# medivhna/TF_Face_Toolbox

Hardware: NVIDIA B200
Metric: A-softmax head fwd+bwd samples/sec at C=85,742 D=512, 1/2/4/8 B200 (higher is better)
Workload: dtype bf16

## Files before the change

tf_face_toolbox_b200/csrc/asm_api.cu:

```cuda
#include <math.h>
#include <stdio.h>
#include <stdlib.h>
#include <string.h>

#include <new>
#include <vector>

#include "../../include/asoftmax_b200.h"
#include "asm_kernels.cuh"

using namespace asmh;

struct asm_head {
  asm_config cfg;
  int device = 0;
  int num_sms = 148;
  int Cp = 0;
  int NT = 0;
  char* ws = nullptr;
  size_t ws_bytes = 0;
  Step st{};
  size_t dx_part_capacity = 0;
  UmmaMaps maps{};
  int maps_B = -1;
// ... 2 lines not shown
  float* dw_scratch = nullptr;
  bool defer_loss = true;
  bool tc = false;
  UmmaTuning tune{8192, 1024, 2048, 15, 0, 0, 1, 1, 0, 3};
  bool fwd_valid = false;
  cudaStream_t side = nullptr;
  cudaEvent_t ev_fork = nullptr, ev_join = nullptr;
  bool overlap = true;
  int dw_pairs = 0;
  bool pdl = true;
  P2P p2p{};
  bool p2p_ready = false;
  float* Xg = nullptr;
  size_t l2_persist_bytes = 0;
  cudaStream_t l2_stream = nullptr;
  bool l2_set = false;
  int launches = 0;
  bool profiling = false;
  bool phase_profiling = false;
  static constexpr int kMaxMarks = 16;
  cudaEvent_t ev[kMaxMarks + 1] = {};
  const char* mark_name[kMaxMarks] = {};
  int n_marks = 0;
  char err[512];
};

namespace {
thread_local char g_create_err[512] = "";

size_t align_up(size_t v, size_t a) { return (v + a - 1) / a * a; }

struct Layout {
  size_t ylocal, flags, n, inv_n, inv_c, margin, tgt_s, tgt_f, part, stats_local, lse, negoff, gtarget, rcoef, rowloss, counter,
      q_part, G, dx_part, Xb, Wb, Xs, Xg, step_dev, wsq_part, wsq_ticket, total;
  int Cp, NT, MT;
  size_t dx_capacity;
};

bool valid_cfg(const asm_config* c) {
  if (!c) return false;
  if (c->D <= 0 || c->D % 16 != 0) return false;
  if (c->C_total <= 0 || c->C_local <= 0 || c->class_offset < 0) return false;
  if ((long long)c->class_offset + c->C_local > c->C_total) return false;
  if (c->B_max <= 0 || c->m < 1 || c->m > 4) return false;
  if (c->mode != ASM_MODE_FP32 && c->mode != ASM_MODE_BF16) return false;
  if (c->mode == ASM_MODE_BF16 && c->D % 64 != 0) return false;
  if (c->world < 1 || c->rank < 0 || c->rank >= c->world) return false;
  if (c->nccl_comm != nullptr) return false;
  return true;
}

bool use_x3(const asm_config& c) {
  if (c.mode != ASM_MODE_FP32 || c.D % 64 != 0) return false;
  const char* e = getenv("ASM_FP32_SIMT");
  return !(e && atoi(e) != 0);
}
bool use_tc(const asm_config& c) { return c.mode == ASM_MODE_BF16 || use_x3(c); }

Layout make_layout(const asm_config& c, int num_sms) {
  Layout L{};
  const bool tc = use_tc(c);
  const size_t planes = use_x3(c) ? 3 : 1;
  const size_t B = c.B_max, D = c.D;
  L.Cp = (int)align_up(c.C_local, 256);
  L.NT = (L.Cp + 127) / 128;
  if (L.NT < 2 * num_sms) L.NT = 2 * num_sms;
  L.MT = 2 * (int)((B + 127) / 128);
  if (L.MT < 4 * (int)((B + 255) / 256)) L.MT = 4 * (int)((B + 255) / 256);
  const int ks_simt = simt_dx_splits(c.B_max, c.D, L.Cp);
  const int ks_umma = umma_dx_splits(c.B_max, c.D, L.Cp, num_sms, 1);
  const int ks_one = tc ? umma_dx_splits(128, c.D, L.Cp, num_sms, 1)
                        : simt_dx_splits(128, c.D, L.Cp);
  const size_t cap_full = (size_t)(tc ? ks_umma : ks_simt) * B * D;
  const size_t cap_one = (size_t)ks_one * (B < 128 ? B : 128) * D;
  L.dx_capacity = cap_full > cap_one ? cap_full : cap_one;
  size_t off = 0;
  auto take = [&](size_t bytes) { size_t o = off; off = align_up(off + bytes, 256); return o; };
  L.ylocal = take(B * 4);
  L.flags = take(256);
  L.n = take(B * 4);
  L.inv_n = take(B * 4);
  L.inv_c = take((size_t)L.Cp * 4);
  L.margin = take(kMarginRecordFloats * 4);
  L.tgt_s = take(B * 4);
  L.tgt_f = take(B * 4);
  L.part = take(B * (size_t)L.NT * 8);
  L.stats_local = take(3 * B * 4);
  L.lse = take(B * 4);
  L.negoff = take(B * 4);
  L.gtarget = take(B * 4);
  L.rcoef = take(B * 4);
  L.rowloss = take(B * 4);
  L.counter = take(256);
  L.wsq_part = take(((size_t)L.Cp / 32 + 16) * 4);
  L.wsq_ticket = take(256);
  L.q_part = take((size_t)L.MT * L.Cp * 4);
  L.G = take(align_up(B, 64) * (size_t)L.Cp * (c.mode == ASM_MODE_BF16 ? 2 : 4));
  L.dx_part = take(L.dx_capacity * 4);
  if (tc) {
    L.Xb = take(planes * B * D * 2);
    L.Wb = take(planes * D * (size_t)L.Cp * 2);
  } else {
    L.Xs = take(B * D * 4);
  }
  if (c.world > 1) {
    L.Xg = take(B * D * 4);
    L.step_dev = take(256);
  }
  L.total = off;
  return L;
}

int fail(asm_head* h, int code, const char* fmt, const char* detail) {
  char* dst = h ? h->err : g_create_err;
  snprintf(dst, 512, fmt, detail ? detail : "");
  return code;
}

#define CU_TRY(h, expr)                                                         \
  do {                                                                          \
    cudaError_t e__ = (expr);                                                   \
    if (e__ != cudaSuccess) return fail(h, ASM_ERR_CUDA, #expr ": %s", cudaGetErrorString(e__)); \
  } while (0)

void mark(asm_head* h, const char* name, cudaStream_t stream, bool phase_start = true) {
  h->launches += 1;
  if (h->phase_profiling && !phase_start) return;
  if (h->profiling && h->n_marks < asm_head::kMaxMarks) {
    cudaEventRecord(h->ev[h->n_marks], stream);
    h->mark_name[h->n_marks] = name;
    h->n_marks += 1;
  }
}
void mark_end(asm_head* h, cudaStream_t stream) {
  if (h->profiling) cudaEventRecord(h->ev[h->n_marks], stream);
}

int check_launch(asm_head* h, const char* what) {
  cudaError_t e = cudaGetLastError();
  if (e != cudaSuccess) {
    snprintf(h->err, 512, "%s: %s", what, cudaGetErrorString(e));
    return ASM_ERR_CUDA;
  }
  return ASM_OK;
}

bool split_active(const asm_head* h) {
  return h->dw_pairs > 0 && h->overlap && (!h->profiling || h->phase_profiling) && h->side != nullptr && h->tc &&
         (h->tune.cg_mask & 12) == 12;
}
int dw_sms(const asm_head* h) { return split_active(h) ? 2 * h->dw_pairs : h->num_sms; }
int dx_sms(const asm_head* h) { return split_active(h) ? h->num_sms - 2 * h->dw_pairs : h->num_sms; }

Step simt_step(const Step& s) {
  Step t = s;
  if (s.mg.kind != 0) t.X = s.Xs;
  return t;
}

int run_forward(asm_head* h, const float* X, int B, const void* labels, int label_bytes,
                const float* W, float lambda, float* logits, bool want_local_stats,
                cudaStream_t stream, const P2P* tp = nullptr) {
  if (!h) return ASM_ERR_INVALID_ARG;
  if (!X || !labels || !W) return fail(h, ASM_ERR_INVALID_ARG, "null input pointer%s", "");
  if (B <= 0 || B > h->cfg.B_max) return fail(h, ASM_ERR_INVALID_ARG, "B out of range%s", "");
  if (label_bytes != 4 && label_bytes != 8)
    return fail(h, ASM_ERR_INVALID_ARG, "label_bytes must be 4 or 8%s", "");
  if (!(lambda >= 0.f)) return fail(h, ASM_ERR_INVALID_ARG, "lambda must be >= 0%s", "");
  Step& s = h->st;
  s.B = B;
  s.lambda = lambda;
  s.invB = 1.0f / (float)B;
  s.Bp = (int)align_up((size_t)B, 64);
  s.X = X;
  s.W = W;
  s.logits = logits;
  s.l2_hints = (h->tune.l2_hints & 1) ? 1 : 0;
  {
    const int bcg = (h->tune.cg_mask & 2) ? 2 : 1;
    const long long bunits = (long long)(s.Cp / (128 * bcg)) * ((B + 255) / 256);
    s.MT = h->tc ? umma_q_parts(B, umma_tile_width(h->tune, bcg, bunits, h->num_sms), bcg)
                 : (B + kRowTileHost - 1) / kRowTileHost;
  }
  h->launches = 0;
  h->n_marks = 0;
  {
    cudaStreamCaptureStatus cs = cudaStreamCaptureStatusNone;
    cudaStreamIsCapturing(stream, &cs);
    s.pdl = (h->pdl && !h->profiling && cs == cudaStreamCaptureStatusNone) ? 1 : 0;
  }
  h->fwd_valid = false;
  if (h->l2_persist_bytes && h->cfg.mode == ASM_MODE_BF16 && (!h->l2_set || h->l2_stream != stream)) {
    cudaDeviceSetLimit(cudaLimitPersistingL2CacheSize, h->l2_persist_bytes);
    cudaStreamAttrValue av{};
    const size_t wb_bytes = (size_t)s.D * s.Cp * 2;
    av.accessPolicyWindow.base_ptr = (void*)s.Wb;
    av.accessPolicyWindow.num_bytes = wb_bytes;
    av.accessPolicyWindow.hitRatio =
        wb_bytes <= h->l2_persist_bytes ? 1.0f : (float)h->l2_persist_bytes / (float)wb_bytes;
    av.accessPolicyWindow.hitProp = cudaAccessPropertyPersisting;
    av.accessPolicyWindow.missProp = cudaAccessPropertyStreaming;
    if (cudaStreamSetAttribute(stream, cudaStreamAttributeAccessPolicyWindow, &av) != cudaSuccess)
      cudaGetLastError();
    h->l2_set = true;
    h->l2_stream = stream;
  }
  if (h->tc) {
    if ((B + 127) / 128 > h->num_sms)
      return fail(h, ASM_ERR_INVALID_ARG, "batch too large for the tcgen05 forward grid%s", "");
    {
      const int fcg = (h->tune.cg_mask & 1) ? 2 : 1;
      const int ecg = (fcg == 2 && B > 128) ? 2 : 1;
      const long long funits = (long long)(((B + 127) / 128 + ecg - 1) / ecg) * (s.Cp / 256);
      s.NT = umma_forward_tiles(B, s.Cp, h->num_sms, fcg, umma_tile_width(h->tune, ecg, funits, h->num_sms));
    }
    s.KS = umma_dx_splits(B, s.D, s.Cp, dx_sms(h), (h->tune.cg_mask & 8) ? 2 : 1);
    while (s.KS > 1 && (size_t)s.KS * B * s.D > h->dx_part_capacity) --s.KS;
    if (h->maps_B != B || h->maps_KS != s.KS) {
      if (!umma_build_maps(&h->maps, s))
        return fail(h, ASM_ERR_CUDA, "cuTensorMapEncodeTiled failed%s", "");
      h->maps_B = B;
      h->maps_KS = s.KS;
    }
  } else {
    s.NT = simt_forward_tiles(s.C);
    s.KS = simt_dx_splits(B, s.D, s.Cp);
  }
  while (s.KS > 1 && (size_t)s.KS * B * s.D > h->dx_part_capacity) --s.KS;
  mark(h, "prep_norms", stream);
  launch_prep(s, labels, label_bytes, stream, tp);
  mark(h, "fwd_logits_stats", stream);
  if (h->tc) launch_umma_forward(s, h->maps, h->tune, h->num_sms, stream);
  else launch_simt_forward(simt_step(s), stream);
  if (want_local_stats) {
    mark(h, "combine_local", stream);
    launch_combine_local(s, stream);
  }
  mark_end(h, stream);
  int rc = check_launch(h, "forward launch");
  if (rc == ASM_OK) h->fwd_valid = true;
  return rc;
}

int run_backward(asm_head* h, const float* stats_all, int n_shards, float* loss_out,
                 float* dX, float* dW, bool grads, cudaStream_t stream, const P2P* tp = nullptr) {
  Step& s = h->st;
  s.loss = loss_out;
  s.dX = dX;
  s.dW = dW;
  s.Wmut = const_cast<float*>(s.W);
  const bool tc = h->tc;
  s.defer_loss = (grads && tc && h->defer_loss) ? 1 : 0;
  if (tp) {
    mark(h, "combine_exchange", stream);
    launch_combine_p2p(s, *tp, stream);
  } else if (stats_all) {
    if (h->profiling && h->n_marks > 0 && h->n_marks < asm_head::kMaxMarks)
      h->mark_name[h->n_marks++] = "stats_exchange_host";
    mark(h, "combine_global", stream);
    launch_combine_global(s, stats_all, n_shards, stream);
  } else {
    mark(h, "combine_stats", stream);
    launch_combine_fused(s, stream);
  }
  if (grads) {
    h->tune.side_by_side = split_active(h) ? 1 : 0;
    mark(h, "bwd_recompute_g", stream);
    if (tc) launch_umma_bwdg(s, h->maps, h->tune, h->num_sms, stream);
    else launch_simt_bwdg(simt_step(s), stream);
    const bool dx_first = !tc && s.opt.kind != 0;
    const bool fork = h->overlap && (!h->profiling || h->phase_profiling) && h->side != nullptr && !dx_first;
    cudaStream_t sx = stream;
    if (fork) {
      cudaEventRecord(h->ev_fork, stream);
      cudaStreamWaitEvent(h->side, h->ev_fork, 0);
      sx = h->side;
    }
    auto run_dx = [&]() {
      mark(h, "dx_gemm", sx, !h->phase_profiling);
      if (tc) launch_umma_dx(s, h->maps, h->tune, dx_sms(h), sx);
      else launch_simt_dx(simt_step(s), sx);
      const bool add = s.mg.kind != 0;
      mark(h, tp ? (add ? "dx_finish_margin_exchange" : "dx_finish_exchange") : (add ? "dx_finish_margin" : "dx_finish"), sx,
           !h->phase_profiling);
      if (tp) launch_dx_finish_p2p(s, *tp, sx);
      else launch_dx_finish(s, sx);
    };
    if (dx_first) run_dx();
    mark(h, h->phase_profiling ? "dw+dx+dx_finish (side by side)" : "dw_gemm", stream);
    if (tc && s.opt.kind != 0 && h->opt_stream) {
      if (!h->dw_scratch &&
          cudaMalloc(&h->dw_scratch, (size_t)s.D * h->cfg.C_local * sizeof(float)) != cudaSuccess) {
        cudaGetLastError();
        h->dw_scratch = nullptr;
// ... 102 lines not shown
    ce = umma_configure();
    if (ce != cudaSuccess) {
      fail(nullptr, ASM_ERR_CUDA, "cudaFuncSetAttribute(smem): %s", cudaGetErrorString(ce));
      cudaFree(h->ws);
      delete h;
      return ASM_ERR_CUDA;
    }
  }
  Step& s = h->st;
  s.D = cfg->D;
  s.C = cfg->C_local;
  s.Cp = L.Cp;
  s.C_total = cfg->C_total;
  s.class_offset = cfg->class_offset;
  s.m = cfg->m;
  s.mode = cfg->mode;
  s.x3 = use_x3(*cfg) ? 1 : 0;
  char* w = h->ws;
  s.ylocal = (int*)(w + L.ylocal);
  s.flags = (int*)(w + L.flags);
  s.n = (float*)(w + L.n);
  s.inv_n = (float*)(w + L.inv_n);
  s.inv_c = (float*)(w + L.inv_c);
  s.tgt_s = (float*)(w + L.tgt_s);
  s.tgt_f = (float*)(w + L.tgt_f);
  s.part = (float2*)(w + L.part);
  s.stats_local = (float*)(w + L.stats_local);
  s.lse = (float*)(w + L.lse);
  s.negoff = (float*)(w + L.negoff);
  s.gtarget = (float*)(w + L.gtarget);
  s.rcoef = (float*)(w + L.rcoef);
  s.rowloss = (float*)(w + L.rowloss);
  s.counter = (unsigned int*)(w + L.counter);
  s.q_part = (float*)(w + L.q_part);
  s.wsq_part = (float*)(w + L.wsq_part);
  s.wsq_ticket = (unsigned int*)(w + L.wsq_ticket);
  s.gscale = 1.0f;
  s.wd_g = 0.0f;
  s.reg_scale = 0.0f;
  s.reg_out = nullptr;
  s.G = (void*)(w + L.G);
  s.dx_part = (float*)(w + L.dx_part);
  h->dx_part_capacity = L.dx_capacity;
  if (h->tc) {
    s.Xb = (__nv_bfloat16*)(w + L.Xb);
    s.Wb = (__nv_bfloat16*)(w + L.Wb);
  } else {
    s.Xs = (float*)(w + L.Xs);
  }
  s.mg.kind = 0;
  if (cfg->world > 1) {
    h->Xg = (float*)(w + L.Xg);
    h->p2p.step_dev = (unsigned*)(w + L.step_dev);
    h->p2p.err_dev = h->p2p.step_dev + 1;
    h->p2p.tickets = h->p2p.step_dev + 2;
  }
  h->Cp = L.Cp;
  *out = h;
  return ASM_OK;
}

int asm_destroy(asm_head* h) {
  if (!h) return ASM_ERR_INVALID_ARG;
  if (h->ws) cudaFree(h->ws);
  if (h->dw_scratch) cudaFree(h->dw_scratch);
  if (h->side) cudaStreamDestroy(h->side);
  if (h->ev_fork) cudaEventDestroy(h->ev_fork);
  if (h->ev_join) cudaEventDestroy(h->ev_join);
  if (h->ev[0])
    for (int i = 0; i <= asm_head::kMaxMarks; ++i) cudaEventDestroy(h->ev[i]);
  delete h;
  return ASM_OK;
}

const char* asm_last_error(const asm_head* h) { return h ? h->err : g_create_err; }

int asm_last_launch_count(const asm_head* h) { return h ? h->launches : 0; }

int asm_forward_partial(asm_head* h, const float* X, int32_t B, const void* labels,
                        int32_t label_bytes, const float* W, float lambda, float* stats_out,
                        float* logits_out_or_null, void* cuda_stream) {
  cudaStream_t stream = (cudaStream_t)cuda_stream;
  int rc = run_forward(h, X, B, labels, label_bytes, W, lambda, logits_out_or_null, true, stream);
  if (rc != ASM_OK) return rc;
  if (!stats_out) return fail(h, ASM_ERR_INVALID_ARG, "stats_out is NULL%s", "");
  CU_TRY(h, cudaMemcpyAsync(stats_out, h->st.stats_local, (size_t)3 * B * sizeof(float),
                            cudaMemcpyDeviceToDevice, stream));
  return ASM_OK;
}

int asm_backward_partial(asm_head* h, const float* stats_all, int32_t n_shards, float* loss_out,
                         float* dX_partial, float* dW, void* cuda_stream) {
  if (!h) return ASM_ERR_INVALID_ARG;
  if (!h->fwd_valid)
    return fail(h, ASM_ERR_INVALID_ARG, "asm_backward_partial without asm_forward_partial%s", "");
  if (!stats_all || n_shards < 1 || !dX_partial || (!dW && h->st.opt.kind == 0))
    return fail(h, ASM_ERR_INVALID_ARG, "null pointer / bad n_shards%s", "");
  return run_backward(h, stats_all, n_shards, loss_out, dX_partial, dW, true,
                      (cudaStream_t)cuda_stream);
}

int asm_forward_backward(asm_head* h, const float* X, int32_t B, const void* labels,
                         int32_t label_bytes, const float* W, float lambda, float* loss_out,
                         float* logits_out_or_null, float* dX, float* dW, void* cuda_stream) {
  cudaStream_t stream = (cudaStream_t)cuda_stream;
  if (h && h->cfg.C_local != h->cfg.C_total)
    return fail(h, ASM_ERR_INVALID_ARG,
                "asm_forward_backward needs a shard that owns every class; use the partial calls%s", "");
  int rc = run_forward(h, X, B, labels, label_bytes, W, lambda, logits_out_or_null, false, stream);
  if (rc != ASM_OK) return rc;
  if (!loss_out || !dX || (!dW && h->st.opt.kind == 0))
    return fail(h, ASM_ERR_INVALID_ARG, "null output pointer%s", "");
  return run_backward(h, nullptr, 1, loss_out, dX, dW, true, stream);
}

int asm_forward(asm_head* h, const float* X, int32_t B, const void* labels, int32_t label_bytes,
                const float* W, float lambda, float* loss_out, float* logits_out_or_null,
                void* cuda_stream) {
  cudaStream_t stream = (cudaStream_t)cuda_stream;
  if (h && h->cfg.C_local != h->cfg.C_total)
    return fail(h, ASM_ERR_INVALID_ARG, "asm_forward needs a shard that owns every class%s", "");
  int rc = run_forward(h, X, B, labels, label_bytes, W, lambda, logits_out_or_null, false, stream);
  if (rc != ASM_OK) return rc;
  if (!loss_out) return fail(h, ASM_ERR_INVALID_ARG, "loss_out is NULL%s", "");
  return run_backward(h, nullptr, 1, loss_out, nullptr, nullptr, false, stream);
}

namespace {
struct P2PLayout { size_t off_x, off_y, off_st, off_dx, off_fl, total; int b_max; };
P2PLayout p2p_layout(const asm_config& c) {
  P2PLayout L{};
  const size_t B = c.B_max, D = c.D;
  L.b_max = (int)((B + c.world - 1) / c.world);
  size_t off = 0;
  auto take = [&](size_t bytes) { size_t o = off; off = align_up(off + bytes, 256); return o; };
  L.off_x = take(2 * (size_t)L.b_max * D * 4);
  L.off_y = take(2 * (size_t)L.b_max * 4);
  L.off_st = take(2 * 3 * B * 4);
  L.off_dx = take(2 * B * D * 4);
  L.off_fl = take(3 * kFlagStride * 4);
  L.total = off;
  return L;
}
}

size_t asm_p2p_bytes(const asm_config* cfg) {
  if (!valid_cfg(cfg) || cfg->world < 2 || cfg->world > kMaxPeers) return 0;
  return p2p_layout(*cfg).total;
}

int asm_p2p_attach(asm_head* h, void* const* peer_bases) {
  if (!h || !peer_bases) return ASM_ERR_INVALID_ARG;
  if (h->cfg.world < 2 || h->cfg.world > kMaxPeers)
    return fail(h, ASM_ERR_INVALID_ARG, "asm_p2p_attach needs 2..8 ranks%s", "");
  const P2PLayout L = p2p_layout(h->cfg);
// ... 8 lines not shown
    if (!peer_bases[r]) return fail(h, ASM_ERR_INVALID_ARG, "peer base is NULL%s", "");
    p.base[r] = (char*)peer_bases[r];
  }
  const char* e = getenv("ASM_P2P_TIMEOUT_MS");
  p.timeout_ns = (unsigned long long)(e ? atoll(e) : 60000ll) * 1000000ull;
  e = getenv("ASM_P2P_WAITERS");
  p.waiters = e ? atoi(e) : 1 << 20;
  if (p.waiters < 1) p.waiters = 1;
  p2p_preload_kernels();
  h->p2p_ready = true;
  return ASM_OK;
}

int asm_step_p2p(asm_head* h, const float* X_local, int32_t b_local, const void* labels_local,
                 int32_t label_bytes, const float* W, float lambda, float* loss_out,
                 float* dX_local, float* dW, void* cuda_stream) {
  if (!h) return ASM_ERR_INVALID_ARG;
  if (!h->p2p_ready) return fail(h, ASM_ERR_INVALID_ARG, "asm_step_p2p before asm_p2p_attach%s", "");
  if (!X_local || !labels_local || !W || !loss_out || !dX_local || (!dW && h->st.opt.kind == 0))
    return fail(h, ASM_ERR_INVALID_ARG, "null pointer%s", "");
  if (label_bytes != 4 && label_bytes != 8)
    return fail(h, ASM_ERR_INVALID_ARG, "label_bytes must be 4 or 8%s", "");
  P2P& p = h->p2p;
  if (b_local <= 0 || b_local > p.b_max || (long long)b_local * p.world > h->cfg.B_max)
    return fail(h, ASM_ERR_INVALID_ARG, "b_local out of range%s", "");
  cudaStream_t stream = (cudaStream_t)cuda_stream;
  p.b_local = b_local;
  p.x_local = X_local;
  p.y_local = labels_local;
  p.y_bytes = label_bytes;
  p.dx_local = dX_local;
  p.Xg = h->Xg;
  const int B = b_local * p.world;
  int rc = run_forward(h, h->Xg, B, labels_local, label_bytes, W, lambda, nullptr, false, stream, &p);
  if (rc == ASM_OK) rc = run_backward(h, nullptr, p.world, loss_out, nullptr, dW, true, stream, &p);
  return rc;
}

int asm_p2p_set_timeout(asm_head* h, int32_t milliseconds) {
  if (!h || milliseconds < 0) return ASM_ERR_INVALID_ARG;
  h->p2p.timeout_ns = (unsigned long long)milliseconds * 1000000ull;
  return ASM_OK;
}

int asm_p2p_status(asm_head* h, void* cuda_stream) {
  if (!h) return ASM_ERR_INVALID_ARG;
  if (!h->p2p_ready) return ASM_OK;
  unsigned code = 0;
  CU_TRY(h, cudaMemcpyAsync(&code, h->p2p.err_dev, sizeof(code), cudaMemcpyDeviceToHost,
                            (cudaStream_t)cuda_stream));
  CU_TRY(h, cudaStreamSynchronize((cudaStream_t)cuda_stream));
  if (code == 0) return ASM_OK;
  snprintf(h->err, sizeof(h->err), "peer %u did not publish phase %u in time (ranks must stay in lock-step)",
           code & 0xffu, (code >> 8) & 0xffu);
  return ASM_ERR_PEER_TIMEOUT;
}

int asm_set_optimizer(asm_head* h, const asm_optimizer* opt, float* state0, float* state1) {
  if (!h) return ASM_ERR_INVALID_ARG;
  Step& s = h->st;
  if (!opt || opt->kind == ASM_OPT_NONE) {
    s.opt.kind = 0;
    s.opt_s0 = s.opt_s1 = nullptr;
    return ASM_OK;
  }
  if (opt->kind != ASM_OPT_MOMENTUM && opt->kind != ASM_OPT_ADAM)
    return fail(h, ASM_ERR_INVALID_ARG, "unknown optimizer kind%s", "");
// ... 112 lines not shown
```

tf_face_toolbox_b200/csrc/asm_kernels.cuh:

```cuda
#pragma once
#include <cuda.h>
#include <cuda_bf16.h>
#include <cuda_runtime.h>
#include <stdint.h>

#include "asm_common.cuh"

namespace asmh {

struct OptParams {
  int kind;
  float lr;
  float mu, b1, b2, eps, wd;
};
__host__ __device__ inline void opt_apply(const OptParams& o, float grad, float& w, float& s0,
                                          float& s1) {
  const float g = grad + o.wd * w;
  if (o.kind == 1) {
    s0 = o.mu * s0 + g;
    w -= o.lr * s0;
  } else {
    s0 = o.b1 * s0 + (1.0f - o.b1) * g;
    s1 = o.b2 * s1 + (1.0f - o.b2) * g * g;
#ifdef __CUDA_ARCH__
// ... 70 lines not shown
struct Step {
  int B, D, C, Cp, C_total, class_offset, m, mode;
  float lambda, invB;
  const float* lambda_dev;
  float gscale;
  float wd_g;
  float reg_scale;
  float* reg_out;
  float* wsq_part;
  unsigned int* wsq_ticket;
  const float* X;
  int x_bf16;
  const float* W;
  float* logits;
  float* dX;
  float* dW;
  float* loss;
  int* ylocal;
  int* flags;
  float* n;
  float* inv_n;
  float* inv_c;
  float* tgt_s;
  float* tgt_f;
  float2* part;
  int NT;
  float* stats_local;
  float* lse;
  float* negoff;
  float* gtarget;
  float* rcoef;
  float* rowloss;
  unsigned int* counter;
  float* q_part;
  int MT;
  void* G;
  int Bp;
  float* dx_part;
  int KS;
  __nv_bfloat16* Xb;
  __nv_bfloat16* Wb;
  int x3;
  OptParams opt;
  float* Wmut;
  float* opt_s0;
  float* opt_s1;
  int l2_hints;
  int pdl;
  int defer_loss;
  Margin mg;
  float* Xs;
};

void launch_prep(const Step& s, const void* labels, int label_bytes, cudaStream_t st, const P2P* p = nullptr);
void launch_combine_p2p(const Step& s, const P2P& p, cudaStream_t st);
void launch_dx_finish_p2p(const Step& s, const P2P& p, cudaStream_t st);
void launch_combine_local(const Step& s, cudaStream_t st);
void launch_combine_global(const Step& s, const float* stats_all, int n_shards, cudaStream_t st);
void launch_combine_fused(const Step& s, cudaStream_t st);
void launch_dx_finish(const Step& s, cudaStream_t st);
void launch_opt_stream(const Step& s, const float* dW, cudaStream_t st);

void p2p_preload_kernels();
void prep_preload_kernels();
void simt_preload_kernels();

// ... 58 lines not shown
```

tf_face_toolbox_b200/csrc/asm_prep.cu:

```cuda
#include <stdlib.h>

#include "asm_common.cuh"
#include "asm_kernels.cuh"
#include "asm_p2p.cuh"
#include "asm_rows.cuh"

namespace asmh {

__device__ __forceinline__ void prep_row_tail(const Step& s, int row, float acc, long long y) {
  const float nn = sqrtf(acc);
  s.n[row] = nn;
  s.inv_n[row] = nn > 0.f ? 1.0f / nn : 0.f;
  const long long yl = y - s.class_offset;
  s.ylocal[row] = (y < 0 || y >= s.C_total) ? -2 : ((yl >= 0 && yl < s.C) ? (int)yl : -1);
  s.tgt_s[row] = 0.f;
  s.tgt_f[row] = 0.f;
}

template <int PL>
__device__ __forceinline__ void prep_row_scaled(const Step& s, const char* x, char* xg, int esz, bool gather,
                                                int row, long long y) {
  const int tx = threadIdx.x & 31;
  const float4* x4 = reinterpret_cast<const float4*>(x);
  const int n16 = s.D * esz / 16;
// ... 281 lines not shown
    if (vec2) prep_kernel<true, 0, TX, TY, U, ADD><<<grd, 256, 0, st>>>(s, labels, label_bytes, nwb, npub, pp);
    else prep_kernel<false, 0, TX, TY, U, ADD><<<grd, 256, 0, st>>>(s, labels, label_bytes, nwb, npub, pp);
  }
}

template <int TX, int TY, int U>
static void launch_prep_t(const Step& s, const void* labels, int label_bytes, cudaStream_t st, const P2P* p) {
  if (s.mg.kind != 0) launch_prep_t<TX, TY, U, true>(s, labels, label_bytes, st, p);
  else launch_prep_t<TX, TY, U, false>(s, labels, label_bytes, st, p);
}

void launch_prep(const Step& s, const void* labels, int label_bytes, cudaStream_t st, const P2P* p) {
  static int shape = -1, small_auto = -1;
  if (shape < 0) {
    const char* e = getenv("ASM_PREP_SHAPE");
    shape = e ? atoi(e) : 0;
    e = getenv("ASM_PREP_AUTO");
    small_auto = (e && atoi(e) != 0) ? 1 : 0;
  }
  if (shape == 0 && small_auto && s.Cp <= 32768) {
    launch_prep_t<16, 16, 8>(s, labels, label_bytes, st, p);
    return;
  }
  if (shape == 1) launch_prep_t<32, 8, 16>(s, labels, label_bytes, st, p);
  else if (shape == 2) launch_prep_t<16, 16, 8>(s, labels, label_bytes, st, p);
  else if (shape == 3) launch_prep_t<128, 2, 16>(s, labels, label_bytes, st, p);
  else launch_prep_t<32, 8, 4>(s, labels, label_bytes, st, p);
}

__global__ void __launch_bounds__(256) combine_local_kernel(Step s) {
  pdl_trigger();
  pdl_wait();
  const int row = blockIdx.x * 8 + (threadIdx.x >> 5);
  const int lane = threadIdx.x & 31;
  if (row >= s.B) return;
  float m = -INFINITY, z = 0.f;
  const float2* p = s.part + (size_t)row * s.NT;
  for (int t = lane; t < s.NT; t += 32) {
    const float2 v = p[t];
    ms_combine(m, z, v.x, v.y);
  }
#pragma unroll
  for (int o = 16; o > 0; o >>= 1) {
    const float m2 = __shfl_xor_sync(0xffffffffu, m, o);
    const float z2 = __shfl_xor_sync(0xffffffffu, z, o);
    ms_combine(m, z, m2, z2);
  }
  if (lane == 0) {
    float* st = s.stats_local;
    st[row] = m;
    st[s.B + row] = z;
    st[2 * s.B + row] = s.ylocal[row] >= 0 ? s.tgt_f[row] : 0.f;
  }
}

void launch_combine_local(const Step& s, cudaStream_t st) {
  launch_pdl(combine_local_kernel, dim3((s.B + 7) / 8), dim3(256), 0, st, s.pdl != 0, 1, s);
}

template <bool FUSED>
__global__ void __launch_bounds__(256) combine_kernel(Step s, const float* stats_all, int n_shards) {
  __shared__ float red[256];
  __shared__ bool is_last;
  pdl_trigger();
  pdl_wait();
  const int row = blockIdx.x * 8 + (threadIdx.x >> 5);
  const int lane = threadIdx.x & 31;
  if (row < s.B) {
    float m = -INFINITY, z = 0.f, fy = 0.f;
    const int yl_row = s.ylocal[row];
    const float tgt_f_row = s.tgt_f[row], tgt_s_row = s.tgt_s[row], inv_n_row = s.inv_n[row];
    if (FUSED) {
      const float2* p = s.part + (size_t)row * s.NT;
      for (int t = lane; t < s.NT; t += 32) {
        const float2 v = p[t];
        ms_combine(m, z, v.x, v.y);
      }
    } else {
      for (int g = lane; g < n_shards; g += 32) {
        const float* sg = stats_all + (size_t)g * 3 * s.B;
        ms_combine(m, z, sg[row], sg[s.B + row]);
        fy += sg[2 * s.B + row];
      }
    }
#pragma unroll
    for (int o = 16; o > 0; o >>= 1) {
      const float m2 = __shfl_xor_sync(0xffffffffu, m, o);
      const float z2 = __shfl_xor_sync(0xffffffffu, z, o);
      ms_combine(m, z, m2, z2);
      fy += __shfl_xor_sync(0xffffffffu, fy, o);
    }
    if (lane == 0) {
      if (FUSED) {
        fy = yl_row >= 0 ? tgt_f_row : 0.f;
        s.stats_local[row] = m;
        s.stats_local[s.B + row] = z;
        s.stats_local[2 * s.B + row] = fy;
      }
      row_epilogue(s, row, m, z, fy, yl_row, tgt_f_row, tgt_s_row, inv_n_row);
    }
  }
  if (s.defer_loss) return;
  last_block_loss(s, red, &is_last);
}

void launch_combine_global(const Step& s, const float* stats_all, int n_shards, cudaStream_t st) {
  launch_pdl(combine_kernel<false>, dim3((s.B + 7) / 8), dim3(256), 0, st, false, 1, s, stats_all, n_shards);
}

void launch_combine_fused(const Step& s, cudaStream_t st) {
  launch_pdl(combine_kernel<true>, dim3((s.B + 7) / 8), dim3(256), 0, st, s.pdl != 0, 1, s,
             static_cast<const float*>(nullptr), 1);
}

template <int KS_T>
__global__ void __launch_bounds__(256) dx_finish_kernel(Step s) {
  pdl_trigger();
  pdl_wait();
  dx_finish_rows<KS_T>(s, s.dX, blockIdx.x, gridDim.x);
}

__global__ void __launch_bounds__(256) dx_finish_margin_kernel(Step s) {
  __shared__ float red[8];
  pdl_trigger();
  pdl_wait();
  dx_finish_rows_margin(s, s.dX, blockIdx.x, gridDim.x, red);
}

void launch_dx_finish(const Step& s, cudaStream_t st) {
  if (s.mg.kind != 0) {
    int blocks = (s.B + 1) / 2;
    if (blocks > 148 * 8) blocks = 148 * 8;
    launch_pdl(dx_finish_margin_kernel, dim3(blocks), dim3(256), 0, st, s.pdl != 0, 1, s);
// ... 95 lines not shown
```

tf_face_toolbox_b200/csrc/asm_rows.cuh:

```cuda
#pragma once
#include "asm_common.cuh"
#include "asm_kernels.cuh"

namespace asmh {

__device__ __forceinline__ void row_epilogue(const Step& s, int row, float m, float z, float fy,
                                             int yl_row, float tgt_f_row, float tgt_s_row,
                                             float inv_n_row) {
  const bool owned = yl_row >= 0;
  const float lse = m + logf(z);
  s.lse[row] = lse;
  const float gB = s.invB * s.gscale;
  s.negoff[row] = -lse * 1.4426950408889634f + log2f(gB);
  s.rowloss[row] = yl_row == -2 ? __int_as_float(0x7fc00000) : lse - fy;
  float gt = 0.f, r = 0.f;
  if (owned && s.mg.kind != 0) {
    float phi, dphi;
    phi_eval(tgt_s_row * s.mg.inv_s, s.mg, phi, dphi);
    gt = (expf(tgt_f_row - lse) - 1.0f) * gB * dphi;
  } else if (owned) {
    float psi, dpsi;
    const float t = fminf(1.f, fmaxf(-1.f, tgt_s_row * inv_n_row));
    psi_eval(t, s.m, psi, dpsi);
    const float gy = (expf(tgt_f_row - lse) - 1.0f) * gB;
    const float lam = step_lambda(s.lambda, s.lambda_dev);
    const float il = 1.0f / (1.0f + lam);
    gt = gy * (lam + dpsi) * il;
    r = gy * (psi - t * dpsi) * il * inv_n_row;
  }
  s.gtarget[row] = gt;
  s.rcoef[row] = r;
}

__device__ __forceinline__ float4 load_x4(const Step& s, size_t i) {
  if (s.x_bf16) {
    const uint2 h = __ldg(reinterpret_cast<const uint2*>(s.X) + i);
    const __nv_bfloat162 a2 = *reinterpret_cast<const __nv_bfloat162*>(&h.x);
    const __nv_bfloat162 b2 = *reinterpret_cast<const __nv_bfloat162*>(&h.y);
    return make_float4(__low2float(a2), __high2float(a2), __low2float(b2), __high2float(b2));
  }
  return __ldg(reinterpret_cast<const float4*>(s.X) + i);
}

template <int KS_T>
__device__ __forceinline__ void dx_finish_rows(const Step& s, float* dxo, unsigned vb, unsigned nb) {
  const size_t total4 = (size_t)s.B * s.D / 4;
  const size_t stride4 = total4;
  for (size_t i = vb * (size_t)blockDim.x + threadIdx.x; i < total4; i += (size_t)nb * blockDim.x) {
    const int row = (int)((i * 4) / s.D);
    const float4* p = reinterpret_cast<const float4*>(s.dx_part) + i;
    const float r = s.rcoef[row];
    const float4 x = load_x4(s, i);
    float4 a = make_float4(r * x.x, r * x.y, r * x.z, r * x.w);
    if (KS_T > 0) {
      float4 v[KS_T > 0 ? KS_T : 1];
#pragma unroll
      for (int z = 0; z < KS_T; ++z) v[z] = __ldcg(p + (size_t)z * stride4);
#pragma unroll
      for (int z = 0; z < KS_T; ++z) { a.x += v[z].x; a.y += v[z].y; a.z += v[z].z; a.w += v[z].w; }
    } else {
      int z = 0;
      for (; z + 4 <= s.KS; z += 4) {
        const float4 v0 = __ldcg(p + (size_t)(z + 0) * stride4);
        const float4 v1 = __ldcg(p + (size_t)(z + 1) * stride4);
        const float4 v2 = __ldcg(p + (size_t)(z + 2) * stride4);
        const float4 v3 = __ldcg(p + (size_t)(z + 3) * stride4);
// ... 115 lines not shown
```

tf_face_toolbox_b200/csrc/asm_umma_gemm.cu:

```cuda
#include <type_traits>

#include "asm_common.cuh"
#include "asm_kernels.cuh"
#include "asm_umma.cuh"

#ifdef ASM_BRINGUP
#define ASM_DBG(flags, bit) ((flags) & (bit))
#else
#define ASM_DBG(flags, bit) 0
#endif

namespace asmh {

namespace {
constexpr int BM = 128, BN = 256, BK = 64, STAGES = 4;
constexpr int BN_FULL = BN;
constexpr int A_BYTES = BM * BK * 2;
constexpr int B_BYTES = BN * BK * 2;
constexpr int STAGE_BYTES = A_BYTES + B_BYTES;
constexpr int AUX_BARS = 512;
constexpr int AUX_VEC = 3 * 2 * BN * 4;
constexpr int STG_HALF = 32 * 128 * 2;
constexpr int AUX_STG = 2 * STG_HALF;
constexpr int WB_BUF = 32 * 128 * 2;
constexpr int AUX_WB = 2 * 2 * WB_BUF;
constexpr int DSTG = 32 * 128 * 4;
constexpr int AUX_REGION = (AUX_VEC + AUX_STG) > AUX_WB ? (AUX_VEC + AUX_STG) : AUX_WB;
constexpr float LOG2E = 1.4426950408889634f;

enum { U_FWD = 0, U_BWDG = 1, U_DW = 2, U_DX = 3, U_FWDR = 4, U_DWOPT = 5, U_DWF = 6, U_BWDG1 = 7 };

#ifndef ASM_FWD_EPI16
#define ASM_FWD_EPI16 1
#endif
constexpr bool FWD_EPI16 = ASM_FWD_EPI16 != 0;
#ifndef ASM_BWDG_EPI16
// ... 16 lines not shown
  static constexpr int CH_B = 64 * KB * 2;
  static constexpr int PIPE_B = RES_B + NST * ST_B;
  static constexpr int AUX_R = (RES || KIND == U_FWD) ? AUX_VEC
                               : (KIND == U_DW ? 2 * NWB * WB_BUF + (DW_TMA ? 4 * DSTG : 0)
                                               : (NSB == 2 ? AUX_VEC + 2 * AUX_STG + (EPIW == 16 ? 2048 : 0) : AUX_REGION));
  static constexpr int SMEM = PIPE_B + AUX_BARS + AUX_R + 1024;
  static_assert(SMEM <= 232448, "exceeds the 227 KB shared memory of an sm_100 CTA");
};

__device__ __forceinline__ void named_bar_sync(int id, int nthreads) {
  asm volatile("bar.sync %0, %1;" ::"r"(id), "r"(nthreads) : "memory");
}
__device__ __forceinline__ float fast_ex2(float x) {
  float y;
  asm("ex2.approx.ftz.f32 %0, %1;" : "=f"(y) : "f"(x));
  return y;
}
__device__ __forceinline__ float sel_eq(int i, int k, float a, float b) {
  float r;
  asm("{\n\t.reg .pred p;\n\tsetp.eq.s32 p, %1, %2;\n\tselp.f32 %0, %3, %4, p;\n\t}\n"
      : "=f"(r)
      : "r"(i), "r"(k), "f"(a), "f"(b));
  return r;
}
__device__ __noinline__ float fwd_target(float* tgt_s, float* tgt_f, const float* n,
                                         const float* inv_n, int m, float lambda, int row,
                                         float sv) {
  tgt_s[row] = sv;
  const Margin mg = *margin_record(tgt_s);
  const float fv = mg.kind != 0 ? additive_logit(sv, mg) : target_logit(sv, n[row], inv_n[row], m, lambda);
  tgt_f[row] = fv;
  return fv;
}
}

template <int KIND, int CG = 1, int BNT = BN_FULL>
__global__ void __launch_bounds__((Geo<KIND, CG, BNT>::NTHREADS), 1)
umma_kernel(const __grid_constant__ CUtensorMap mapA, const __grid_constant__ CUtensorMap mapB,
            const __grid_constant__ CUtensorMap mapC, const __grid_constant__ CUtensorMap mapD,
            const __grid_constant__ CUtensorMap mapE, Step s, UmmaArgs g) {
  using G_ = Geo<KIND, CG, BNT>;
  constexpr int BN = BNT;
  constexpr int EPIW = G_::EPIW;
  constexpr int NQ = EPIW / 4;
  constexpr int HC = BN / NQ;
  constexpr int EPI_THREADS = 32 * EPIW;
  static_assert(BNT == 256 || BNT == 128, "tile width");
  static_assert(BNT == 256 || (KIND != U_FWDR && KIND != U_BWDG1), "narrow tiles: main kinds only");
  pdl_trigger();
  const int crank = CG == 2 ? (int)ptx::cluster_ctarank() : 0;
  const int pair_id = (int)blockIdx.x / CG;
  const int npairs = (int)gridDim.x / CG;
  constexpr bool IS_FWD = (KIND == U_FWD || KIND == U_FWDR);
  constexpr bool RES = G_::RES;
  constexpr int KB = G_::KB, NST = G_::NST, A_ST = G_::A_ST, ST_B = G_::ST_B;
  constexpr int RES_B = G_::RES_B, CH_B = G_::CH_B, PIPE_B = G_::PIPE_B;
  constexpr bool IS_DW = (KIND == U_DW || KIND == U_DWOPT || KIND == U_DWF);
  constexpr bool IS_BWDG = (KIND == U_BWDG || KIND == U_BWDG1);
  constexpr bool A_MN = (IS_BWDG || KIND == U_DX);
  constexpr bool B_MN = (IS_FWD || IS_DW);
  constexpr bool N_FAST = (IS_BWDG || IS_DW);
  extern __shared__ uint8_t smem_raw[];
  uint8_t* smem = smem_raw + ((1024u - (ptx::smem_u32(smem_raw) & 1023u)) & 1023u);
  uint8_t* pipe = smem + RES_B;
  uint64_t* full = reinterpret_cast<uint64_t*>(smem + PIPE_B);
  uint64_t* empty = full + 8;
  uint64_t* tfull = empty + 8;
  uint64_t* tempty = tfull + 2;
  uint64_t* wfull = tempty + 2;
  uint64_t* wempty = wfull + 8;
  uint64_t* sfull = wempty + 8;
  uint64_t* sempty = sfull + 4;
  uint32_t* tmem_ptr = reinterpret_cast<uint32_t*>(sempty + 4);
// ... 238 lines not shown
              ptx::tma_store_2d(&mapD, src, m0, db >> 1);
              ptx::tma_store_2d(&mapE, src + DSTG / 2, s.C + m0 + dw_sh, db >> 1);
            }
            ptx::bulk_commit();
            ptx::bulk_wait_read0();
          }
          ptx::mbar_arrive(&sempty[half * 2 + sb]);
        }
      }
      ptx::bulk_wait0();
    }
  } else if (warp == 3) {
    if (KIND == U_DW && !ASM_DBG(g.debug_flags, 1) && ptx::elect_one()) {
      uint32_t cc = 0;
      for (int u = pair_id; u < total; u += npairs) {
        int z, m_idx, n_idx;
        decode(u, z, m_idx, n_idx);
        m_idx = m_idx * CG + crank;
        for (int c = 0; c < BN / 64; ++c, ++cc) {
          const uint32_t buf = cc % NWB, ph = (cc / NWB) & 1;
#pragma unroll
          for (int h = 0; h < 2; ++h) {
            ptx::mbar_wait(&wempty[h * NWB + buf], ph ^ 1);
            ptx::mbar_expect_tx(&wfull[h * NWB + buf], WB_BUF);
            const int d0 = n_idx * BN + h * HC + c * 32;
#pragma unroll
            for (int qb = 0; qb < 2; ++qb)
              ptx::tma_load_2d(wbuf + (h * NWB + buf) * WB_BUF + qb * (WB_BUF / 2), &mapC, &wfull[h * NWB + buf], 0,
                               ((m_idx * BM + qb * 64) >> 6) * s.D + d0);
          }
        }
      }
    }
    if (KIND == U_DX && s.defer_loss && blockIdx.x == 0) {
      float part[8];
#pragma unroll
      for (int v = 0; v < 8; ++v) {
        float acc = 0.f;
        for (int i = v * 32 + lane; i < s.B; i += 256) acc += __ldcg(s.rowloss + i);
        part[v] = acc;
      }
#pragma unroll
      for (int o = 4; o > 0; o >>= 1)
#pragma unroll
        for (int v = 0; v < o; ++v) part[v] += part[v + o];
      float r = part[0];
#pragma unroll
      for (int o = 16; o > 0; o >>= 1) r += __shfl_down_sync(0xffffffffu, r, o);
      if (lane == 0 && s.loss) *s.loss = r * s.invB;
    }
  } else if (warp >= 4) {
    const int q4 = warp & 3;
    const int half = (warp - 4) >> 2;
    const int et = threadIdx.x - 128;
    const int lane_row = q4 * 32 + lane;
    const int col0 = half * HC;
    uint32_t lt = 0;
    float pre0 = 0.f, pre1 = 0.f, pre2 = 0.f, pre3 = 0.f, pre4 = 0.f, pre5 = 0.f;
    float run_m = -INFINITY, run_z = 0.f;
    int fwd_row = -1;
    auto prefetch_tile = [&](int pu) {
      if (pu >= total) return;
      int pz, pm, pn;
      decode(pu, pz, pm, pn);
      pm = pm * CG + crank;
      if (IS_FWD) pre0 = s.inv_c[pn * BN + (et & (BN - 1))];
      if (IS_BWDG) {
        const int i = pn * BN + (et & (BN - 1));
        const bool iv = i < s.B;
        pre0 = iv ? s.negoff[i] : -INFINITY;
        pre1 = iv ? __int_as_float(s.ylocal[i]) : __int_as_float(-1);
        pre2 = iv ? s.gtarget[i] : 0.f;
        pre3 = s.inv_c[pm * BM + lane_row];
      }
      if (IS_DW) {
        const int pj = pm * BM + lane_row;
        const float* qp = s.q_part + pj;
        pre0 = qp[0];
        pre1 = s.MT > 1 ? qp[(size_t)s.Cp] : 0.f;
        pre2 = s.inv_c[pj];
        pre3 = s.MT > 2 ? qp[(size_t)2 * s.Cp] : 0.f;
        pre4 = s.MT > 3 ? qp[(size_t)3 * s.Cp] : 0.f;
        pre5 = 0.f;
// ... 436 lines not shown
          } else if (rv && n0 + col0 + c * 32 < s.D) {
#pragma unroll
            for (int b = 0; b < 32; b += 4)
              *reinterpret_cast<float4*>(out + c * 32 + b) =
                  make_float4(__uint_as_float(r[b]), __uint_as_float(r[b + 1]),
                              __uint_as_float(r[b + 2]), __uint_as_float(r[b + 3]));
          }
        };
        ASM_EPILOGUE_CHUNKS(process)
      }
#undef ASM_EPILOGUE_CHUNKS
    }
    if (IS_BWDG && EPIW == 16 && lt > 0) {
      named_bar_sync(1, EPI_THREADS);
      if (q_prev_idx >= 0 && (half & 1) == 0)
        s.q_part[q_prev_idx] = q_prev + qx[(q_prev_a * 2 + (half >> 1)) * 128 + lane_row];
    }
#ifdef ASM_TIMING
    if ((pair_id == 0 || pair_id == npairs / 2) && crank == 0 && lane == 0 && (warp == 4 || warp == 11))
      printf("TIMING kind %d pair %d warp %d: epilogue total %lld cyc, wait tfull %lld\n", KIND, pair_id, warp,
             clock64() - e_all, e_wait);
#endif
    if (IS_FWD && fwd_row >= 0)
      s.part[(size_t)fwd_row * s.NT + (pair_id / g.mt) * NQ + half] = make_float2(run_m, run_z);
  }

  if ((IS_BWDG || KIND == U_DX) && warp >= 4 && lane == 0) ptx::bulk_wait0();
  ptx::tc_fence_before();
  __syncthreads();
  if (CG == 2) ptx::cluster_sync_all();
  if (warp == 2) {
    if (CG == 2) ptx::tmem_dealloc_cg2(tmem_base, 512); else ptx::tmem_dealloc(tmem_base, 512);
  }
}

namespace {
typedef CUresult (*EncodeTiledFn)(CUtensorMap*, CUtensorMapDataType, cuuint32_t, void*,
                                  const cuuint64_t*, const cuuint64_t*, const cuuint32_t*,
                                  const cuuint32_t*, CUtensorMapInterleave, CUtensorMapSwizzle,
                                  CUtensorMapL2promotion, CUtensorMapFloatOOBfill);
EncodeTiledFn get_encode_fn() {
  static EncodeTiledFn fn = nullptr;
  if (fn) return fn;
  void* p = nullptr;
  cudaDriverEntryPointQueryResult qres;
  if (cudaGetDriverEntryPoint("cuTensorMapEncodeTiled", &p, cudaEnableDefault, &qres) !=
          cudaSuccess ||
      qres != cudaDriverEntryPointSuccess)
    return nullptr;
  fn = reinterpret_cast<EncodeTiledFn>(p);
  return fn;
}

bool encode_map(CUtensorMap* m, const void* base, uint64_t inner, uint64_t outer, uint64_t pitch,
                uint32_t box_inner, uint32_t box_outer, bool swizzle128 = true, bool f32 = false,
                bool swizzle64 = false) {
  EncodeTiledFn fn = get_encode_fn();
  if (!fn) return false;
  cuuint64_t dims[2] = {inner, outer};
  cuuint64_t strides[1] = {pitch * (f32 ? 4 : 2)};
  cuuint32_t box[2] = {box_inner, box_outer};
  cuuint32_t estr[2] = {1, 1};
  return fn(m, f32 ? CU_TENSOR_MAP_DATA_TYPE_FLOAT32 : CU_TENSOR_MAP_DATA_TYPE_BFLOAT16, 2,
            const_cast<void*>(base), dims, strides, box,
            estr, CU_TENSOR_MAP_INTERLEAVE_NONE,
            swizzle128 ? CU_TENSOR_MAP_SWIZZLE_128B
// ... 283 lines not shown
```

Before: 2.181 million.

## Fold per-row softmax stats combine into forward UMMA kernel via row tickets

The forward UMMA kernel now takes a per-row-block ticket when it finishes. The last CTA for each row block merges the partial (max, sum) pairs for those rows and writes the stats, and in the full fwd+bwd path it also computes the row epilogue and the mean loss. This removes the separate combine_local and combine_fused kernel launches and their extra pass over the partials. The cost is atomic ticket traffic and a serialized tail on the last CTA of each row block. It also needs ticket counters that are reset between calls, and the diff does not show where that reset happens.

After: 2.127 million (median of 6 runs). -2.5%, worse.

```diff
diff --git a/tf_face_toolbox_b200/csrc/asm_api.cu b/tf_face_toolbox_b200/csrc/asm_api.cu
--- a/tf_face_toolbox_b200/csrc/asm_api.cu
+++ b/tf_face_toolbox_b200/csrc/asm_api.cu
@@ -58,7 +58,7 @@
 
 struct Layout {
   size_t ylocal, flags, n, inv_n, inv_c, margin, tgt_s, tgt_f, part, stats_local, lse, negoff, gtarget, rcoef, rowloss, counter,
-      q_part, G, dx_part, Xb, Wb, Xs, Xg, step_dev, wsq_part, wsq_ticket, total;
+      row_tickets, q_part, G, dx_part, Xb, Wb, Xs, Xg, step_dev, wsq_part, wsq_ticket, total;
   int Cp, NT, MT;
   size_t dx_capacity;
 };
@@ -118,6 +118,7 @@
   L.rcoef = take(B * 4);
   L.rowloss = take(B * 4);
   L.counter = take(256);
+  L.row_tickets = take(((B + 127) / 128 + 2) * 4);
   L.wsq_part = take(((size_t)L.Cp / 32 + 16) * 4);
   L.wsq_ticket = take(256);
   L.q_part = take((size_t)L.MT * L.Cp * 4);
@@ -184,8 +185,14 @@
   return t;
 }
 
+enum class After {
+  kExchange,
+  kLocalStats,
+  kCombine,
+};
+
 int run_forward(asm_head* h, const float* X, int B, const void* labels, int label_bytes,
-                const float* W, float lambda, float* logits, bool want_local_stats,
+                const float* W, float lambda, float* logits, After after, bool grads, float* loss_out,
                 cudaStream_t stream, const P2P* tp = nullptr) {
   if (!h) return ASM_ERR_INVALID_ARG;
   if (!X || !labels || !W) return fail(h, ASM_ERR_INVALID_ARG, "null input pointer%s", "");
@@ -202,6 +209,11 @@
   s.W = W;
   s.logits = logits;
   s.l2_hints = (h->tune.l2_hints & 1) ? 1 : 0;
+  s.fold = !h->tc ? 0 : after == After::kCombine ? 2 : after == After::kLocalStats ? 1 : 0;
+  if (s.fold == 2) {
+    s.defer_loss = (grads && h->defer_loss) ? 1 : 0;
+    s.loss = loss_out;
+  }
   {
     const int bcg = (h->tune.cg_mask & 2) ? 2 : 1;
     const long long bunits = (long long)(s.Cp / (128 * bcg)) * ((B + 255) / 256);
@@ -258,7 +270,7 @@
   mark(h, "fwd_logits_stats", stream);
   if (h->tc) launch_umma_forward(s, h->maps, h->tune, h->num_sms, stream);
   else launch_simt_forward(simt_step(s), stream);
-  if (want_local_stats) {
+  if (after == After::kLocalStats && !s.fold) {
     mark(h, "combine_local", stream);
     launch_combine_local(s, stream);
   }
@@ -285,7 +297,7 @@
       h->mark_name[h->n_marks++] = "stats_exchange_host";
     mark(h, "combine_global", stream);
     launch_combine_global(s, stats_all, n_shards, stream);
-  } else {
+  } else if (!s.fold) {
     mark(h, "combine_stats", stream);
     launch_combine_fused(s, stream);
   }
@@ -454,6 +466,7 @@
   s.rcoef = (float*)(w + L.rcoef);
   s.rowloss = (float*)(w + L.rowloss);
   s.counter = (unsigned int*)(w + L.counter);
+  s.row_tickets = (unsigned int*)(w + L.row_tickets);
   s.q_part = (float*)(w + L.q_part);
   s.wsq_part = (float*)(w + L.wsq_part);
   s.wsq_ticket = (unsigned int*)(w + L.wsq_ticket);
@@ -503,7 +516,7 @@
                         int32_t label_bytes, const float* W, float lambda, float* stats_out,
                         float* logits_out_or_null, void* cuda_stream) {
   cudaStream_t stream = (cudaStream_t)cuda_stream;
-  int rc = run_forward(h, X, B, labels, label_bytes, W, lambda, logits_out_or_null, true, stream);
+  int rc = run_forward(h, X, B, labels, label_bytes, W, lambda, logits_out_or_null, After::kLocalStats, true, nullptr, stream);
   if (rc != ASM_OK) return rc;
   if (!stats_out) return fail(h, ASM_ERR_INVALID_ARG, "stats_out is NULL%s", "");
   CU_TRY(h, cudaMemcpyAsync(stats_out, h->st.stats_local, (size_t)3 * B * sizeof(float),
@@ -529,7 +542,7 @@
   if (h && h->cfg.C_local != h->cfg.C_total)
     return fail(h, ASM_ERR_INVALID_ARG,
                 "asm_forward_backward needs a shard that owns every class; use the partial calls%s", "");
-  int rc = run_forward(h, X, B, labels, label_bytes, W, lambda, logits_out_or_null, false, stream);
+  int rc = run_forward(h, X, B, labels, label_bytes, W, lambda, logits_out_or_null, After::kCombine, true, loss_out, stream);
   if (rc != ASM_OK) return rc;
   if (!loss_out || !dX || (!dW && h->st.opt.kind == 0))
     return fail(h, ASM_ERR_INVALID_ARG, "null output pointer%s", "");
@@ -542,7 +555,7 @@
   cudaStream_t stream = (cudaStream_t)cuda_stream;
   if (h && h->cfg.C_local != h->cfg.C_total)
     return fail(h, ASM_ERR_INVALID_ARG, "asm_forward needs a shard that owns every class%s", "");
-  int rc = run_forward(h, X, B, labels, label_bytes, W, lambda, logits_out_or_null, false, stream);
+  int rc = run_forward(h, X, B, labels, label_bytes, W, lambda, logits_out_or_null, After::kCombine, false, loss_out, stream);
   if (rc != ASM_OK) return rc;
   if (!loss_out) return fail(h, ASM_ERR_INVALID_ARG, "loss_out is NULL%s", "");
   return run_backward(h, nullptr, 1, loss_out, nullptr, nullptr, false, stream);
@@ -617,7 +630,7 @@
   p.dx_local = dX_local;
   p.Xg = h->Xg;
   const int B = b_local * p.world;
-  int rc = run_forward(h, h->Xg, B, labels_local, label_bytes, W, lambda, nullptr, false, stream, &p);
+  int rc = run_forward(h, h->Xg, B, labels_local, label_bytes, W, lambda, nullptr, After::kExchange, true, nullptr, stream, &p);
   if (rc == ASM_OK) rc = run_backward(h, nullptr, p.world, loss_out, nullptr, dW, true, stream, &p);
   return rc;
 }
diff --git a/tf_face_toolbox_b200/csrc/asm_kernels.cuh b/tf_face_toolbox_b200/csrc/asm_kernels.cuh
--- a/tf_face_toolbox_b200/csrc/asm_kernels.cuh
+++ b/tf_face_toolbox_b200/csrc/asm_kernels.cuh
@@ -126,6 +126,8 @@
   float* rcoef;
   float* rowloss;
   unsigned int* counter;
+  int fold;
+  unsigned int* row_tickets;
   float* q_part;
   int MT;
   void* G;
diff --git a/tf_face_toolbox_b200/csrc/asm_prep.cu b/tf_face_toolbox_b200/csrc/asm_prep.cu
--- a/tf_face_toolbox_b200/csrc/asm_prep.cu
+++ b/tf_face_toolbox_b200/csrc/asm_prep.cu
@@ -337,26 +337,8 @@
   pdl_trigger();
   pdl_wait();
   const int row = blockIdx.x * 8 + (threadIdx.x >> 5);
-  const int lane = threadIdx.x & 31;
-  if (row >= s.B) return;
-  float m = -INFINITY, z = 0.f;
-  const float2* p = s.part + (size_t)row * s.NT;
-  for (int t = lane; t < s.NT; t += 32) {
-    const float2 v = p[t];
-    ms_combine(m, z, v.x, v.y);
-  }
-#pragma unroll
-  for (int o = 16; o > 0; o >>= 1) {
-    const float m2 = __shfl_xor_sync(0xffffffffu, m, o);
-    const float z2 = __shfl_xor_sync(0xffffffffu, z, o);
-    ms_combine(m, z, m2, z2);
-  }
-  if (lane == 0) {
-    float* st = s.stats_local;
-    st[row] = m;
-    st[s.B + row] = z;
-    st[2 * s.B + row] = s.ylocal[row] >= 0 ? s.tgt_f[row] : 0.f;
-  }
+  const int rows[1] = {row < s.B ? row : -1};
+  combine_rows<false, 1>(s, rows);
 }
 
 void launch_combine_local(const Step& s, cudaStream_t st) {
@@ -371,22 +353,17 @@
   pdl_wait();
   const int row = blockIdx.x * 8 + (threadIdx.x >> 5);
   const int lane = threadIdx.x & 31;
-  if (row < s.B) {
+  if (FUSED) {
+    const int rows[1] = {row < s.B ? row : -1};
+    combine_rows<true, 1>(s, rows);
+  } else if (row < s.B) {
     float m = -INFINITY, z = 0.f, fy = 0.f;
     const int yl_row = s.ylocal[row];
     const float tgt_f_row = s.tgt_f[row], tgt_s_row = s.tgt_s[row], inv_n_row = s.inv_n[row];
-    if (FUSED) {
-      const float2* p = s.part + (size_t)row * s.NT;
-      for (int t = lane; t < s.NT; t += 32) {
-        const float2 v = p[t];
-        ms_combine(m, z, v.x, v.y);
-      }
-    } else {
-      for (int g = lane; g < n_shards; g += 32) {
-        const float* sg = stats_all + (size_t)g * 3 * s.B;
-        ms_combine(m, z, sg[row], sg[s.B + row]);
-        fy += sg[2 * s.B + row];
-      }
+    for (int g = lane; g < n_shards; g += 32) {
+      const float* sg = stats_all + (size_t)g * 3 * s.B;
+      ms_combine(m, z, sg[row], sg[s.B + row]);
+      fy += sg[2 * s.B + row];
     }
 #pragma unroll
     for (int o = 16; o > 0; o >>= 1) {
@@ -395,15 +372,7 @@
       ms_combine(m, z, m2, z2);
       fy += __shfl_xor_sync(0xffffffffu, fy, o);
     }
-    if (lane == 0) {
-      if (FUSED) {
-        fy = yl_row >= 0 ? tgt_f_row : 0.f;
-        s.stats_local[row] = m;
-        s.stats_local[s.B + row] = z;
-        s.stats_local[2 * s.B + row] = fy;
-      }
-      row_epilogue(s, row, m, z, fy, yl_row, tgt_f_row, tgt_s_row, inv_n_row);
-    }
+    if (lane == 0) row_epilogue(s, row, m, z, fy, yl_row, tgt_f_row, tgt_s_row, inv_n_row);
   }
   if (s.defer_loss) return;
   last_block_loss(s, red, &is_last);
diff --git a/tf_face_toolbox_b200/csrc/asm_rows.cuh b/tf_face_toolbox_b200/csrc/asm_rows.cuh
--- a/tf_face_toolbox_b200/csrc/asm_rows.cuh
+++ b/tf_face_toolbox_b200/csrc/asm_rows.cuh
@@ -32,6 +32,89 @@
   s.rcoef[row] = r;
 }
 
+template <bool FULL, int R>
+__device__ __forceinline__ void combine_rows(const Step& s, const int (&rows)[R]) {
+  static_assert(R >= 1 && R <= 32, "one row per finishing lane");
+  const int lane = threadIdx.x & 31;
+  int row = -1;
+#pragma unroll
+  for (int k = 0; k < R; ++k)
+    if (lane == k) row = rows[k];
+  int yl = 0;
+  float tf = 0.f, ts = 0.f, in = 0.f;
+  if (row >= 0) {
+    yl = s.ylocal[row];
+    tf = __ldcg(s.tgt_f + row);
+    if (FULL) {
+      ts = __ldcg(s.tgt_s + row);
+      in = s.inv_n[row];
+    }
+  }
+  float m[R], z[R];
+#pragma unroll
+  for (int r = 0; r < R; ++r) {
+    m[r] = -INFINITY;
+    z[r] = 0.f;
+  }
+  float2 v[R];
+#pragma unroll
+  for (int r = 0; r < R; ++r)
+    if (rows[r] >= 0 && lane < s.NT) v[r] = __ldcg(s.part + (size_t)rows[r] * s.NT + lane);
+#pragma unroll 1
+  for (int t = lane; t < s.NT; t += 32) {
+    float2 w[R];
+#pragma unroll
+    for (int r = 0; r < R; ++r)
+      if (rows[r] >= 0 && t + 32 < s.NT) w[r] = __ldcg(s.part + (size_t)rows[r] * s.NT + t + 32);
+#pragma unroll
+    for (int r = 0; r < R; ++r) {
+      if (rows[r] >= 0) ms_combine(m[r], z[r], v[r].x, v[r].y);
+      v[r] = w[r];
+    }
+  }
+#pragma unroll 1
+  for (int o = 16; o > 0; o >>= 1) {
+#pragma unroll
+    for (int r = 0; r < R; ++r) {
+      const float m2 = __shfl_xor_sync(0xffffffffu, m[r], o);
+      const float z2 = __shfl_xor_sync(0xffffffffu, z[r], o);
+      ms_combine(m[r], z[r], m2, z2);
+    }
+  }
+  float mr = m[0], zr = z[0];
+#pragma unroll
+  for (int k = 1; k < R; ++k)
+    if (lane == k) {
+      mr = m[k];
+      zr = z[k];
+    }
+  if (row < 0) return;
+  const float fy = yl >= 0 ? tf : 0.f;
+  s.stats_local[row] = mr;
+  s.stats_local[s.B + row] = zr;
+  s.stats_local[2 * s.B + row] = fy;
+  if (FULL) row_epilogue(s, row, mr, zr, fy, yl, tf, ts, in);
+}
+
+__device__ __forceinline__ void mean_loss_warp(const Step& s) {
+  const int lane = threadIdx.x & 31;
+  float part[8];
+#pragma unroll
+  for (int v = 0; v < 8; ++v) {
+    float acc = 0.f;
+    for (int i = v * 32 + lane; i < s.B; i += 256) acc += __ldcg(s.rowloss + i);
+    part[v] = acc;
+  }
+#pragma unroll
+  for (int o = 4; o > 0; o >>= 1)
+#pragma unroll
+    for (int v = 0; v < o; ++v) part[v] += part[v + o];
+  float r = part[0];
+#pragma unroll
+  for (int o = 16; o > 0; o >>= 1) r += __shfl_down_sync(0xffffffffu, r, o);
+  if (lane == 0 && s.loss) *s.loss = r * s.invB;
+}
+
 __device__ __forceinline__ float4 load_x4(const Step& s, size_t i) {
   if (s.x_bf16) {
     const uint2 h = __ldg(reinterpret_cast<const uint2*>(s.X) + i);
diff --git a/tf_face_toolbox_b200/csrc/asm_umma_gemm.cu b/tf_face_toolbox_b200/csrc/asm_umma_gemm.cu
--- a/tf_face_toolbox_b200/csrc/asm_umma_gemm.cu
+++ b/tf_face_toolbox_b200/csrc/asm_umma_gemm.cu
@@ -2,6 +2,8 @@
 
 #include "asm_common.cuh"
 #include "asm_kernels.cuh"
+#include "asm_p2p.cuh"
+#include "asm_rows.cuh"
 #include "asm_umma.cuh"
 
 #ifdef ASM_BRINGUP
@@ -84,13 +86,33 @@
   tgt_f[row] = fv;
   return fv;
 }
+__device__ __noinline__ void fwd_fold_combine(const Step& s, int mt, int cg) {
+  const int crank = cg == 2 ? (int)ptx::cluster_ctarank() : 0;
+  const int rb = ((int)blockIdx.x / cg % mt) * cg + crank;
+  const unsigned nctas = gridDim.x / cg / mt, nrb = mt * cg;
+  if (block_ticket(s.row_tickets + rb, nctas) != nctas - 1) return;
+  __threadfence();
+  const int warp = threadIdx.x >> 5, nw = blockDim.x >> 5;
+  const int r_end = min(s.B, (rb + 1) * BM);
+  for (int r0 = rb * BM + warp; r0 < r_end; r0 += 4 * nw) {
+    int rows[4];
+#pragma unroll
+    for (int k = 0; k < 4; ++k) rows[k] = r0 + k * nw < r_end ? r0 + k * nw : -1;
+    if (s.fold == 2) combine_rows<true, 4>(s, rows);
+    else combine_rows<false, 4>(s, rows);
+  }
+  if (s.fold != 2 || s.defer_loss) return;
+  if (block_ticket(s.row_tickets + nrb, nrb) != nrb - 1) return;
+  __threadfence();
+  if (warp == 0) mean_loss_warp(s);
+}
 }
 
 template <int KIND, int CG = 1, int BNT = BN_FULL>
 __global__ void __launch_bounds__((Geo<KIND, CG, BNT>::NTHREADS), 1)
 umma_kernel(const __grid_constant__ CUtensorMap mapA, const __grid_constant__ CUtensorMap mapB,
             const __grid_constant__ CUtensorMap mapC, const __grid_constant__ CUtensorMap mapD,
-            const __grid_constant__ CUtensorMap mapE, Step s, UmmaArgs g) {
+            const __grid_constant__ CUtensorMap mapE, const __grid_constant__ Step s, UmmaArgs g) {
   using G_ = Geo<KIND, CG, BNT>;
   constexpr int BN = BNT;
   constexpr int EPIW = G_::EPIW;
@@ -395,23 +417,7 @@
         }
       }
     }
-    if (KIND == U_DX && s.defer_loss && blockIdx.x == 0) {
-      float part[8];
-#pragma unroll
-      for (int v = 0; v < 8; ++v) {
-        float acc = 0.f;
-        for (int i = v * 32 + lane; i < s.B; i += 256) acc += __ldcg(s.rowloss + i);
-        part[v] = acc;
-      }
-#pragma unroll
-      for (int o = 4; o > 0; o >>= 1)
-#pragma unroll
-        for (int v = 0; v < o; ++v) part[v] += part[v + o];
-      float r = part[0];
-#pragma unroll
-      for (int o = 16; o > 0; o >>= 1) r += __shfl_down_sync(0xffffffffu, r, o);
-      if (lane == 0 && s.loss) *s.loss = r * s.invB;
-    }
+    if (KIND == U_DX && s.defer_loss && blockIdx.x == 0) mean_loss_warp(s);
   } else if (warp >= 4) {
     const int q4 = warp & 3;
     const int half = (warp - 4) >> 2;
@@ -914,6 +920,8 @@
   if (warp == 2) {
     if (CG == 2) ptx::tmem_dealloc_cg2(tmem_base, 512); else ptx::tmem_dealloc(tmem_base, 512);
   }
+  if constexpr (IS_FWD)
+    if (s.fold) fwd_fold_combine(s, g.mt, CG);
 }
 
 namespace {
```
